# RichardZJM/lammps-mtp-kokkos

Measured on AMD Instinct MI355X. Metric: atom-steps/s (64k-atom W, level-16 MTP), higher is better.
Workload: dtype f64; 1 GPU; 65536-atom BCC W (a=3.165 A, +-0.05 A jitter, seed 777), W_L16.mtp (B=130 T=894 S=116 A=332 R=8 Mu=4 C=149), rc=5 A, full list 7 A, eflag=1 vflag=1; atoms=65536, potential=W_L16.mtp, parallelism=single GPU, atoms_rank0=65536, list_entries_rank0=5802796

## Files before the change

lammps_mtp_kokkos_amd/csrc/mtp_potential.cpp:

```cpp
#include "mtp_potential.hpp"

#include "../../include/mtp_mi355x.h"

#include <algorithm>
#include <cassert>
#include <cerrno>
#include <cmath>
#include <cstdio>
#include <cstdlib>
#include <cstring>
#include <stdexcept>

#include <unistd.h>

namespace {

struct ParseError {
  int code;
  std::string msg;
};

class LineReader {
 public:
  explicit LineReader(FILE *fp) : fp_(fp), buf_(1024) {}
// ... 80 lines not shown
    if (key != kw) throw ParseError{MTP_ERR_PARSE, msg};
  }
};

void parse_text(FILE *fp, bool want_selection, mtp_potential &p)
{
  LineReader rd(fp);
  Cursor c{rd, {}, {}, {}};

  c.advance(kSeps);
  if (c.key != "MTP") throw ParseError{MTP_ERR_FORMAT, "Only MTP potential files are accepted."};
  {
    std::string ver;
    if (!rd.next(ver) || ver != "version = 1.1.0\n")
      throw ParseError{MTP_ERR_FORMAT, "MTP file must have version \"1.1.0\""};
  }
  c.advance(kSeps);
  if (c.key == "potential_name") {
    std::string w;
    p.potential_name = c.tok.next(w) ? w : "";
    c.advance(kSeps);
  }
  p.scaling = 1.0;
  if (c.key == "scaling") {
    p.scaling = c.tok.real();
    c.advance(kSeps);
  }
  c.expect("species_count", "Error reading MTP file. Species count not found.");
  p.species_count = c.tok.integer();
  if (p.species_count < 1) throw ParseError{MTP_ERR_PARSE, "species_count must be positive"};

  c.advance(kSeps);
  if (c.key == "potential_tag") {
    std::string w;
    p.potential_tag = c.tok.next(w) ? w : "";
    c.advance(kSeps);
  }
  c.expect("radial_basis_type", "Error reading MTP file. No radial basis set type is specified.");
  {
    std::string ty = c.tok.word();
    if (ty != "RBChebyshev")
      throw ParseError{MTP_ERR_UNSUPPORTED,
                       "Error reading MTP file. The specified radial basis set type, " + ty + ", was not found.."};
  }
  c.advance(kSeps);
  if (c.key == "scaling") {
    (void) c.tok.real();
    c.advance(kSeps);
  }
  if (c.key != "min_val" && c.key != "min_dist")
    throw ParseError{MTP_ERR_PARSE, "Error in reading MTP file. Cannot read lower cutoff."};
  p.min_cutoff = c.tok.real();
  c.advance(kSeps);
  if (c.key != "max_val" && c.key != "max_dist")
    throw ParseError{MTP_ERR_PARSE, "Error in reading MTP file. Cannot read upper cutoff."};
  p.max_cutoff = c.tok.real();
  c.advance(kSeps);
  c.expect("radial_basis_size", "Error in reading MTP file. Cannot read radial basis set size.");
  p.radial_basis_size = c.tok.integer();

  c.advance(kSeps);
  c.expect("radial_funcs_count", "Error in reading MTP file. Cannot read radial function count.");
  p.radial_func_count = c.tok.integer();
  c.advance(kSeps);
  if (c.key != "radial_coeffs") {
    if (c.key == "magnetic_basis_type")
      throw ParseError{MTP_ERR_UNSUPPORTED, "Magnetic basis is currently not supported."};
    throw ParseError{MTP_ERR_PARSE, "Error in reading MTP file. Cannot read radial coeffs count."};
  }
  const int Sp = p.species_count, R = p.radial_basis_size, Mu = p.radial_func_count;
  if (R < 1 || Mu < 1) throw ParseError{MTP_ERR_PARSE, "radial basis sizes must be positive"};
  p.radial_basis_coeffs.assign((size_t) Sp * Sp * Mu * R, 0.0);
  p.setflag.assign((size_t) (Sp + 1) * (Sp + 1), 0);
  for (int blk = 0; blk < Sp * Sp; blk++) {
    if (!rd.next(c.line)) throw ParseError{MTP_ERR_EOF, "Unexpected end of MTP file."};
    Tokens hdr(c.line, kSepsDash);
    int t1 = hdr.integer(), t2 = hdr.integer();
    if (t1 < 0 || t2 < 0 || t1 >= Sp || t2 >= Sp)
      throw ParseError{MTP_ERR_PARSE, "radial_coeffs block names a species outside species_count"};
    p.setflag[(size_t) (t1 + 1) * (Sp + 1) + t2 + 1] = 1;
    double *dst = &p.radial_basis_coeffs[(size_t) (t1 * Sp + t2) * Mu * R];
    for (int mu = 0; mu < Mu; mu++) {
      if (!rd.next(c.line)) throw ParseError{MTP_ERR_EOF, "Unexpected end of MTP file."};
      Tokens row(c.line, kSepsBrace);
      for (int ri = 0; ri < R; ri++) dst[mu * R + ri] = row.real();
    }
  }
  c.advance(kSeps);
  c.expect("alpha_moments_count", "Error reading MTP file. Alpha moment count not found.");
  p.alpha_moment_count = c.tok.integer();
  c.advance(kSeps);
  c.expect("alpha_index_basic_count", "Error reading MTP file. Alpha moment count not found.");
  p.alpha_index_basic_count = c.tok.integer();
  const int B = p.alpha_index_basic_count;
  if (B < 1) throw ParseError{MTP_ERR_TABLE, "alpha_index_basic_count must be positive"};

  rd.set_bufsize((size_t) B * 20 + 20);
  c.advance(kSepsBrace);
  c.expect("alpha_index_basic", "Error reading MTP file. Alpha index basic not found.");
  p.alpha_index_basic.resize((size_t) B * 4);
  int mu_max = 0, rank_max = 0;
  for (int i = 0; i < B; i++) {
    int32_t *q = &p.alpha_index_basic[4 * (size_t) i];
    for (int j = 0; j < 4; j++) q[j] = c.tok.integer();
    mu_max = std::max(mu_max, (int) q[0]);
    rank_max = std::max(rank_max, (int) (q[1] + q[2] + q[3]));
  }
  if (mu_max != Mu - 1) throw ParseError{MTP_ERR_TABLE, "Wrong number of radial functions specified!"};
  p.max_alpha_index_basic = rank_max + 1;

  c.advance(kSeps);
  c.expect("alpha_index_times_count", "Error reading MTP file. Alpha index times count not found.");
  p.alpha_index_times_count = c.tok.integer();
  const int T = p.alpha_index_times_count;
  rd.set_bufsize((size_t) std::max(T, 0) * 32 + 20);
  c.advance(kSepsBrace);
  c.expect("alpha_index_times", "Error reading MTP file. Alpha index times not found.");
  p.alpha_index_times.resize((size_t) std::max(T, 0) * 4);
  for (size_t i = 0; i < p.alpha_index_times.size(); i++) p.alpha_index_times[i] = c.tok.integer();

  c.advance(kSeps);
  c.expect("alpha_scalar_moments", "Error reading MTP file. Alpha scalar moment count not found.");
  p.alpha_scalar_count = c.tok.integer();
  const int S = p.alpha_scalar_count;
  c.advance(kSepsBrace);
  c.expect("alpha_moment_mapping", "Error reading MTP file. Alpha moment mappings not found.");
  p.alpha_moment_mapping.resize((size_t) S);
  for (int i = 0; i < S; i++) p.alpha_moment_mapping[i] = c.tok.integer();
  c.advance(kSepsBrace);
  c.expect("species_coeffs", "Error reading MTP file. Species coefficients not found.");
  p.species_coeffs.resize((size_t) Sp);
  for (int i = 0; i < Sp; i++) p.species_coeffs[i] = c.tok.real();
  c.advance(kSepsBrace);
  c.expect("moment_coeffs", "Error reading MTP file. Moment coefficients not found.");
  p.linear_coeffs.resize((size_t) S);
  for (int i = 0; i < S; i++) p.linear_coeffs[i] = c.tok.real();

  p.coeff_count = Sp * Sp * Mu * R + Sp + S;

  if (!want_selection) return;
  rd.ignore_comments = false;
  std::string ln;
  if (!rd.next(ln)) {
    p.selection_absent = true;
    throw ParseError{MTP_ERR_SELECTION,
                     "No selection state found! Consider training/retraining or disabling extrapolation!"};
  }
  {
    Tokens t(ln, kSeps);
    std::string w;
    if (!t.next(w) || w != "#MVS_v1.1")
      throw ParseError{MTP_ERR_SELECTION,
                       "Error in reading MTP file selection state. Please verify MVS version is #MVS_v1.1!"};
  }
  rd.ignore_comments = true;
  int energy_weight = 0, site_en_weight = 0;
  static const char *names[5] = {"energy_weight", "force_weight", "stress_weight", "site_en_weight",
                                 "weight_scaling"};
  for (int w = 0; w < 5; w++) {
    c.advance(kSeps);
    if (c.key != names[w])
      throw ParseError{MTP_ERR_SELECTION, std::string("Error in reading MTP file, ") + names[w]};
    if (w == 0) energy_weight = (int) c.tok.real();
    if (w == 3) site_en_weight = (int) c.tok.real();
  }
  if (energy_weight + site_en_weight > 1)
    throw ParseError{MTP_ERR_MODE,
                     "Error, the MTP currently only supports configuration mode (energy_weight=1) or "
                     "neighbourhood mode (site_en_weight=1). Please retrain the MTP with the correct modes!"};
  p.configuration_mode = (energy_weight == 1);
  const size_t n = (size_t) p.coeff_count * p.coeff_count;
  p.active_set.resize(n);
  p.inverse_active_set.resize(n);
  fgetc(fp);
  p.selection_offset = std::ftell(fp);
  if (fread(p.active_set.data(), sizeof(double), n, fp) != n ||
      fread(p.inverse_active_set.data(), sizeof(double), n, fp) != n)
    throw ParseError{MTP_ERR_IO, "Unexpected end of file while reading the active set"};
  p.has_selection = true;
}

}

int mtp_parse_file(const char *path, bool want_selection, mtp_potential &pot, std::string &err)
{
  const int rc = mtp_parse_text_file(path, want_selection, pot, err);
  return rc == MTP_OK ? pot.finalize(err) : rc;
}

int mtp_parse_text_file(const char *path, bool want_selection, mtp_potential &pot, std::string &err)
{
  FILE *fp = std::fopen(path, "rb");
  if (!fp) {
    err = std::string("Cannot open potential file ") + path + ": " + std::strerror(errno);
    return MTP_ERR_IO;
  }
  int rc = MTP_OK;
  try {
    parse_text(fp, want_selection, pot);
  } catch (const ParseError &e) {
    err = e.msg;
    rc = e.code;
  } catch (const std::exception &e) {
    err = e.what();
    rc = MTP_ERR_PARSE;
  }
  std::fclose(fp);
  return rc;
}

void mtp_build_coeff_tables(const mtp_potential &p, const double *radial, const double *species, const double *moments,
                            mtp_coeff_tables &out)
{
  const int A = p.alpha_moment_count, S = p.alpha_scalar_count;
  const std::vector<int32_t> &perm = p.moment_perm;
  const double *lin = moments ? moments : p.linear_coeffs.data();
  const double *ra = radial ? radial : p.radial_basis_coeffs.data();
  const double *sp = species ? species : p.species_coeffs.data();
  out.radial.assign(ra, ra + p.radial_basis_coeffs.size());
  out.species.assign(sp, sp + p.species_coeffs.size());
  auto is_leaf = [&](int m) { return perm[(size_t) m] >= p.stored_moment_count; };
  std::vector<int> last((size_t) A, -1);
  for (int i = 0; i < S; i++) last[(size_t) p.alpha_moment_mapping[(size_t) i]] = i;
  out.seed_val.clear();
  for (int m = 0; m < A; m++)
    if (last[(size_t) m] >= 0 && !is_leaf(m)) out.seed_val.push_back(lin[last[(size_t) m]]);
  std::vector<double> c_energy((size_t) A, 0.0), c_seed((size_t) A, 0.0);
  out.e_lin.clear();
  for (int i = 0; i < S; i++) {
    const int m = p.alpha_moment_mapping[(size_t) i], ml = perm[(size_t) m];
    if (is_leaf(m)) {
      c_energy[(size_t) ml] += lin[i];
      c_seed[(size_t) ml] = lin[i];
    } else {
      out.e_lin.push_back(lin[i]);
    }
  }
  const size_t leaf_row0 = (size_t) p.level_offset[(size_t) p.normal_levels];
  const size_t nleaf_rows = p.rows_by_level.size() - leaf_row0;
  out.leaf_cf.assign(nleaf_rows, 0.0);
  out.leaf_cb.assign(nleaf_rows, 0.0);
  for (size_t r = 0; r < nleaf_rows; r++) {
    const MtpRow &row = p.rows_by_level[leaf_row0 + r];
    if (row.mult == 0) continue;
    out.leaf_cf[r] = c_energy[(size_t) row.a3] * row.mult;
    out.leaf_cb[r] = c_seed[(size_t) row.a3] * row.mult;
  }
}

int mtp_check_compatible(const mtp_potential &a, const mtp_potential &b, bool want_selection, std::string &err)
{
  auto differ = [&](const std::string &name, const std::string &x, const std::string &y) {
    err = "the new file differs in " + name + ": " + y + ", the loaded potential has " + x;
    return (int) MTP_ERR_UNSUPPORTED;
  };
  auto num = [](double v) {
    char t[40];
    std::snprintf(t, sizeof t, "%.17g", v);
    return std::string(t);
  };
#define MTP_SAME_INT(field, name) \
  if (a.field != b.field) return differ(name, std::to_string(a.field), std::to_string(b.field))
#define MTP_SAME_REAL(field, name) \
  if (!(a.field == b.field)) return differ(name, num(a.field), num(b.field))
  MTP_SAME_REAL(scaling, "scaling");
  MTP_SAME_INT(species_count, "species_count");
  MTP_SAME_REAL(min_cutoff, "min_dist");
  MTP_SAME_REAL(max_cutoff, "max_dist");
  MTP_SAME_INT(radial_basis_size, "radial_basis_size");
  MTP_SAME_INT(radial_func_count, "radial_funcs_count");
  MTP_SAME_INT(alpha_moment_count, "alpha_moments_count");
  MTP_SAME_INT(alpha_index_basic_count, "alpha_index_basic_count");
  MTP_SAME_INT(alpha_index_times_count, "alpha_index_times_count");
  MTP_SAME_INT(alpha_scalar_count, "alpha_scalar_moments");
#undef MTP_SAME_INT
#undef MTP_SAME_REAL
  auto table = [&](const char *name, const std::vector<int32_t> &x, const std::vector<int32_t> &y, size_t width) {
    if (x.size() != y.size()) return differ(name, std::to_string(x.size()) + " entries", std::to_string(y.size()) + " entries");
    for (size_t k = 0; k < x.size(); k++)
      if (x[k] != y[k])
        return differ(std::string(name) + "[" + std::to_string(k / width) + (width > 1 ? "][" + std::to_string(k % width) + "]" : "]"),
                      std::to_string(x[k]), std::to_string(y[k]));
    return (int) MTP_OK;
  };
  int rc = table("alpha_index_basic", a.alpha_index_basic, b.alpha_index_basic, 4);
  if (rc == MTP_OK) rc = table("alpha_index_times", a.alpha_index_times, b.alpha_index_times, 4);
  if (rc == MTP_OK) rc = table("alpha_moment_mapping", a.alpha_moment_mapping, b.alpha_moment_mapping, 1);
  if (rc != MTP_OK) return rc;
  if (want_selection) {
    const char *modes[2] = {"neighbourhood (site_en_weight = 1)", "configuration (energy_weight = 1)"};
    if (a.coeff_count != b.coeff_count) return differ("coeff_count", std::to_string(a.coeff_count), std::to_string(b.coeff_count));
    if (a.has_selection != b.has_selection)
      return differ("selection state", a.has_selection ? "present" : "absent", b.has_selection ? "present" : "absent");
    if (a.configuration_mode != b.configuration_mode)
      return differ("selection mode", modes[a.configuration_mode ? 1 : 0], modes[b.configuration_mode ? 1 : 0]);
  }
  return MTP_OK;
}

namespace {

struct ScheduleOptions {
  bool leaves, renumber, debug_banks;
  int bank_rounds = -1, bank_scale = -1, refine_programs = -1;
};

ScheduleOptions read_options()
{
  ScheduleOptions o;
  o.leaves = !std::getenv("MTP_NO_LEAF");
  o.renumber = !std::getenv("MTP_NO_RENUMBER");
  o.debug_banks = std::getenv("MTP_DEBUG_BANKS") != nullptr;
  if (const char *e = std::getenv("MTP_BANK_ROUNDS")) o.bank_rounds = std::max(0, std::atoi(e));
  if (const char *e = std::getenv("MTP_BANK_SCALE")) o.bank_scale = std::max(1, std::atoi(e));
  if (const char *e = std::getenv("MTP_REFINE_PROGRAMS")) o.refine_programs = std::atoi(e) != 0;
  return o;
}

struct Lcg {
  uint64_t state;
  uint32_t operator()() { return (uint32_t) ((state = state * 6364136223846793005ull + 1442695040888963407ull) >> 33); }
};

int refuse(std::string &err, int code, const char *msg)
{
  err = msg;
  return code;
}

int validate(const mtp_potential &p, std::string &err)
{
  const int A = p.alpha_moment_count, B = p.alpha_index_basic_count, T = p.alpha_index_times_count;
  if (A < B) return refuse(err, MTP_ERR_TABLE, "alpha_moments_count is smaller than alpha_index_basic_count");
  for (int i = 0; i < B; i++) {
    const int32_t *q = &p.alpha_index_basic[4 * (size_t) i];
    if (q[0] < 0 || q[1] < 0 || q[2] < 0 || q[3] < 0)
      return refuse(err, MTP_ERR_TABLE, "negative entry in alpha_index_basic");
    if (q[1] > 15 || q[2] > 15 || q[3] > 15)
      return refuse(err, MTP_ERR_LIMIT, "alpha_index_basic exponent above 15 is not supported");
  }
  if (p.max_alpha_index_basic > 12)
    return refuse(err, MTP_ERR_LIMIT, "tensor rank above 11 is not supported by this build");
  for (int k = 0; k < T; k++) {
    const int32_t *q = &p.alpha_index_times[4 * (size_t) k];
    for (int j : {0, 1, 3})
      if (q[j] < 0 || q[j] >= A)
        return refuse(err, MTP_ERR_TABLE, "alpha_index_times refers to a moment outside alpha_moments_count");
  }
  for (int m : p.alpha_moment_mapping)
    if (m < 0 || m >= A)
      return refuse(err, MTP_ERR_TABLE, "alpha_moment_mapping refers to a moment outside alpha_moments_count");
  for (int i = 0; i < B; i++)
    if (p.alpha_index_basic[4 * (size_t) i] > 15)
      return refuse(err, MTP_ERR_LIMIT, "radial function index above 15 is not supported");
  return MTP_OK;
}

int build_slots(mtp_potential &p, std::string &err)
{
  const int B = p.alpha_index_basic_count, P = p.max_alpha_index_basic, Mu = p.radial_func_count;
  p.slot_of.assign((size_t) Mu * P, -1);
  for (int i = 0; i < B; i++) {
    const int32_t *q = &p.alpha_index_basic[4 * (size_t) i];
    p.slot_of[(size_t) q[0] * P + (q[1] + q[2] + q[3])] = -2;
  }
  p.slot_count = 0;
  p.slot_coef_off.clear();
  p.slot_mu.clear();
  p.coef_total = 0;
  for (int nu = 0; nu < 14; nu++) {
    p.deg_first[nu] = p.slot_count;
    p.deg_coef[nu] = p.coef_total;
    if (nu >= P) continue;
    for (int mu = 0; mu < Mu; mu++)
      if (p.slot_of[(size_t) mu * P + nu] == -2) {
        p.slot_of[(size_t) mu * P + nu] = p.slot_count++;
        p.slot_coef_off.push_back(p.coef_total);
        p.slot_mu.push_back(mu);
        p.coef_total += nu == 0 ? 1 : 3 * (nu * (nu + 1) / 2);
      }
  }
  if (p.slot_count > 256) return refuse(err, MTP_ERR_LIMIT, "more than 256 distinct (mu, nu) radial slots");
  p.basic_pack.resize((size_t) B);
  for (int i = 0; i < B; i++) {
    const int32_t *q = &p.alpha_index_basic[4 * (size_t) i];
    const int s = p.slot_of[(size_t) q[0] * P + (q[1] + q[2] + q[3])];
    p.basic_pack[i] = s | (q[1] << 8) | (q[2] << 12) | (q[3] << 16) | (q[0] << 20);
  }
  if (p.coef_total > 65534)
    return refuse(err, MTP_ERR_LIMIT,
                  "derivative-polynomial coefficient blocks above 65534 entries are not supported by this build");
  p.basic_tgt.assign((size_t) 2 * B, 0);
  std::vector<int> hits((size_t) p.coef_total, 0);
  for (int i = 0; i < B; i++) {
    const int32_t *q = &p.alpha_index_basic[4 * (size_t) i];
    const int a = q[1], b = q[2], c = q[3], j = b + c, nu = a + j, C = nu * (nu + 1) / 2;
    const int base = p.slot_coef_off[(size_t) (p.basic_pack[i] & 255)];
    uint32_t tx = 0xffffu, ty = 0xffffu, tz = 0xffffu, fa = (uint32_t) a;
    if (nu == 0) {
      tx = (uint32_t) base;
      fa = 1;
    }
    if (a > 0) tx = (uint32_t) (base + j * (j + 1) / 2 + c);
    if (b > 0) ty = (uint32_t) (base + C + (j - 1) * j / 2 + c);
    if (c > 0) tz = (uint32_t) (base + 2 * C + (j - 1) * j / 2 + c - 1);
    for (uint32_t t : {tx, ty, tz})
      if (t != 0xffffu) hits[t]++;
    p.basic_tgt[2 * (size_t) i] = (int32_t) (tx | (ty << 16));
    p.basic_tgt[2 * (size_t) i + 1] = (int32_t) (tz | (fa << 16) | ((uint32_t) b << 20) | ((uint32_t) c << 24));
  }
  p.coef_dense = 1;
  for (int t = 0; t < p.coef_total; t++) {
    if (hits[t] > 1) return refuse(err, MTP_ERR_TABLE, "alpha_index_basic lists the same (mu, a, b, c) twice");
    if (hits[t] == 0) p.coef_dense = 0;
  }
  return MTP_OK;
}

int build_blocks(mtp_potential &p, std::string &err)
{
  const int B = p.alpha_index_basic_count, P = p.max_alpha_index_basic, slot_count = p.slot_count;
  std::vector<int> basic_of((size_t) slot_count * 16 * 16 * 16, -1);
  for (int i = 0; i < B; i++) {
    const int32_t *q = &p.alpha_index_basic[4 * (size_t) i];
    basic_of[(((size_t) (p.basic_pack[i] & 255) * 16 + q[1]) * 16 + q[2]) * 16 + q[3]] = i;
  }
  p.fwd_blocks.clear();
  p.fwd_block_count = 0;
  std::vector<int> covered((size_t) B, 0);
  for (int j = 0; j < P; j++) {
    std::vector<std::pair<int, int>> heads, tails;
    for (int nu = j; nu < P; nu++)
      for (int sidx = p.deg_first[nu]; sidx < p.deg_first[nu + 1]; sidx++) heads.push_back({sidx, nu - j});
    for (int c = 0; c <= j; c++) tails.push_back({j - c, c});
    for (size_t h0 = 0; h0 < heads.size(); h0 += 3)
      for (size_t t0 = 0; t0 < tails.size(); t0 += 3) {
        int32_t w[8] = {0, 0, 0, 0, 0, 0, 0, 0};
        int16_t kk[10];
        for (int e = 0; e < 10; e++) kk[e] = -1;
        bool any = false;
        for (int h = 0; h < 3 && h0 + h < heads.size(); h++) {
          w[0] |= heads[h0 + h].first << (8 * h);
          w[1] |= heads[h0 + h].second << (4 * h);
        }
        for (int t = 0; t < 3 && t0 + t < tails.size(); t++) {
          w[1] |= tails[t0 + t].first << (12 + 4 * t);
          w[2] |= tails[t0 + t].second << (4 * t);
        }
        for (int h = 0; h < 3 && h0 + h < heads.size(); h++)
          for (int t = 0; t < 3 && t0 + t < tails.size(); t++) {
            const int k = basic_of[(((size_t) heads[h0 + h].first * 16 + heads[h0 + h].second) * 16 +
                                    tails[t0 + t].first) * 16 + tails[t0 + t].second];
            if (k >= 0) {
              kk[3 * h + t] = (int16_t) k;
              covered[k]++;
              any = true;
            }
          }
        if (!any) continue;
        std::memcpy(&w[3], kk, sizeof(int16_t) * 10);
        p.fwd_blocks.insert(p.fwd_blocks.end(), w, w + 8);
        p.fwd_block_count++;
      }
  }
  for (int i = 0; i < B; i++)
    if (covered[i] != 1)
      return refuse(err, MTP_ERR_TABLE, "internal: basic moment not covered exactly once by the head x tail blocks");
  return MTP_OK;
}

int build_blocks5(mtp_potential &p, std::string &err)
{
  const int B = p.alpha_index_basic_count, P = p.max_alpha_index_basic, slot_count = p.slot_count;
  std::vector<int> basic_of((size_t) slot_count * 16 * 16 * 16, -1);
  for (int i = 0; i < B; i++) {
    const int32_t *q = &p.alpha_index_basic[4 * (size_t) i];
    basic_of[(((size_t) (p.basic_pack[i] & 255) * 16 + q[1]) * 16 + q[2]) * 16 + q[3]] = i;
  }
  p.fwd5_blocks.clear();
  p.fwd5_block_count = 0;
  std::vector<int> covered((size_t) B, 0);
  typedef std::pair<int, int> Pair;
  for (int j = 0; j < P; j++) {
    std::vector<Pair> heads, tails;
    auto basic = [&](const Pair &h, const Pair &t) {
      return basic_of[(((size_t) h.first * 16 + h.second) * 16 + t.first) * 16 + t.second];
    };
    {
      std::vector<Pair> all_heads, all_tails;
      for (int nu = j; nu < P; nu++)
        for (int sidx = p.deg_first[nu]; sidx < p.deg_first[nu + 1]; sidx++) all_heads.push_back({sidx, nu - j});
      for (int c = 0; c <= j; c++) all_tails.push_back({j - c, c});
      for (const Pair &h : all_heads)
        if (std::any_of(all_tails.begin(), all_tails.end(), [&](const Pair &t) { return basic(h, t) >= 0; })) heads.push_back(h);
      for (const Pair &t : all_tails)
        if (std::any_of(heads.begin(), heads.end(), [&](const Pair &h) { return basic(h, t) >= 0; })) tails.push_back(t);
    }
    auto cut = [&](int nh, int nt, std::vector<int32_t> *out) {
      int count = 0;
      for (size_t h0 = 0; h0 < heads.size(); h0 += nh)
        for (size_t t0 = 0; t0 < tails.size(); t0 += nt) {
          const int hf[3] = {0, 1, 2}, tf[3] = {3, 4, 2};
          int32_t w[8] = {0, 0, 0, 0, 0, 0, 0, 0};
          int16_t kk[6] = {-1, -1, -1, -1, -1, -1};
          bool any = false;
          for (int h = 0; h < nh && h0 + h < heads.size(); h++) w[hf[h]] |= heads[h0 + h].first | (heads[h0 + h].second << 16);
          for (int t = 0; t < nt && t0 + t < tails.size(); t++) w[tf[t]] |= tails[t0 + t].first | (tails[t0 + t].second << 16);
          if (nh == 3) w[2] |= (int32_t) 0x80000000u;
          for (int h = 0; h < nh && h0 + h < heads.size(); h++)
            for (int t = 0; t < nt && t0 + t < tails.size(); t++) {
              const int k = basic(heads[h0 + h], tails[t0 + t]);
              if (k < 0) continue;
              const int e = h < 2 && t < 2 ? 2 * h + t : nh == 3 ? 4 + t : 4 + h;
              kk[e] = (int16_t) k;
              if (out) covered[k]++;
              any = true;
            }
          if (!any) continue;
          count++;
          if (out) {
            std::memcpy(&w[5], kk, sizeof kk);
            out->insert(out->end(), w, w + 8);
          }
        }
      return count;
    };
    if (heads.empty()) continue;
    const bool wide = cut(3, 2, nullptr) <= cut(2, 3, nullptr);
    p.fwd5_block_count += wide ? cut(3, 2, &p.fwd5_blocks) : cut(2, 3, &p.fwd5_blocks);
  }
  for (int i = 0; i < B; i++)
    if (covered[i] != 1)
      return refuse(err, MTP_ERR_TABLE, "internal: basic moment not covered exactly once by the five-factor blocks");
  return MTP_OK;
}

std::vector<char> find_leaves(const mtp_potential &p, bool enabled)
{
  const int A = p.alpha_moment_count, B = p.alpha_index_basic_count, T = p.alpha_index_times_count;
  std::vector<char> leaf((size_t) A, 0);
  if (!enabled) return leaf;
  std::vector<char> is_factor((size_t) A, 0), is_target((size_t) A, 0);
  std::vector<int> last_write((size_t) A, -1);
  for (int k = 0; k < T; k++) {
    const int32_t *q = &p.alpha_index_times[4 * (size_t) k];
    is_factor[q[0]] = is_factor[q[1]] = 1;
    is_target[q[3]] = 1;
    last_write[q[3]] = k;
  }
  for (int m = B; m < A; m++) leaf[m] = is_target[m] && !is_factor[m];
  for (int k = 0; k < T; k++) {
    const int32_t *q = &p.alpha_index_times[4 * (size_t) k];
    if (leaf[q[3]] && (last_write[q[0]] > k || last_write[q[1]] > k)) leaf[q[3]] = 0;
  }
  return leaf;
}

void build_levels(mtp_potential &p, const std::vector<char> &leaf)
{
  const int A = p.alpha_moment_count, T = p.alpha_index_times_count;
  std::vector<int> wlevel((size_t) A, 0), rlevel((size_t) A, 0);
  std::vector<int> lvl((size_t) T, 0);
  int nlev = 0;
  for (int k = 0; k < T; k++) {
    const int32_t *q = &p.alpha_index_times[4 * (size_t) k];
    if (leaf[q[3]]) continue;
    int l = std::max(wlevel[q[0]], wlevel[q[1]]) + 1;
    l = std::max(l, rlevel[q[3]] + 1);
    lvl[k] = l;
    wlevel[q[3]] = std::max(wlevel[q[3]], l);
    rlevel[q[0]] = std::max(rlevel[q[0]], l);
    rlevel[q[1]] = std::max(rlevel[q[1]], l);
    nlev = std::max(nlev, l);
  }
  p.normal_levels = nlev;
  nlev++;
  for (int k = 0; k < T; k++)
    if (leaf[p.alpha_index_times[4 * (size_t) k + 3]]) lvl[k] = nlev;
  p.level_offset.assign((size_t) nlev + 1, 0);
  for (int k = 0; k < T; k++) p.level_offset[lvl[k]]++;
  for (int l = 1; l <= nlev; l++) p.level_offset[l] += p.level_offset[l - 1];
  std::vector<int32_t> cur((size_t) nlev + 1, 0);
  for (int l = 1; l <= nlev; l++) cur[l] = p.level_offset[l - 1];
  p.rows_by_level.assign((size_t) T, MtpRow{0, 0, 0, 0});
  for (int k = 0; k < T; k++) {
    const int32_t *q = &p.alpha_index_times[4 * (size_t) k];
    p.rows_by_level[cur[lvl[k]]++] = MtpRow{q[0], q[1], q[2], q[3]};
  }
}

void order_rows(mtp_potential &p)
{
  const int nlev = p.normal_levels + 1;
  for (int l = 1; l <= nlev; l++) {
    const int b = p.level_offset[l - 1], e = p.level_offset[l];
    const int n = e - b;
    if (n <= 16) continue;
    std::vector<MtpRow> pool(p.rows_by_level.begin() + b, p.rows_by_level.begin() + e), out;
    std::vector<char> used((size_t) n, 0);
    out.reserve((size_t) n);
    int remaining = n, scan_from = 0;
    while (remaining > 0) {
      int rd0[32], rd1[32], rd3[32];
      for (int h = 0; h < 2 && remaining > 0; h++) {
        if (h == 0)
          for (int q = 0; q < 32; q++) rd0[q] = rd1[q] = rd3[q] = -1;
        int at0[16], at1[16], at3[16];
        for (int q = 0; q < 16; q++) at0[q] = at1[q] = at3[q] = -1;
        for (int slot = 0; slot < 16 && remaining > 0; slot++) {
          int best = -1, best_cost = 1 << 30;
          int seen = 0;
          for (int k = scan_from; k < n && seen < 256; k++) {
            if (used[k]) continue;
            seen++;
            const MtpRow &r = pool[k];
            int cost = 0;
            cost += (rd0[r.a0 & 31] >= 0 && rd0[r.a0 & 31] != r.a0);
            cost += (rd1[r.a1 & 31] >= 0 && rd1[r.a1 & 31] != r.a1);
            if (l < nlev) {
              cost += (rd3[r.a3 & 31] >= 0 && rd3[r.a3 & 31] != r.a3);
              cost += 2 * (at3[r.a3 & 15] >= 0);
            }
            cost += (at0[r.a0 & 15] >= 0) + (at1[r.a1 & 15] >= 0);
            if (cost < best_cost) {
              best_cost = cost;
              best = k;
              if (cost == 0) break;
            }
          }
          assert(best >= 0);
          const MtpRow &r = pool[best];
          used[best] = 1;
          remaining--;
          while (scan_from < n && used[scan_from]) scan_from++;
          rd0[r.a0 & 31] = r.a0;
          rd1[r.a1 & 31] = r.a1;
          rd3[r.a3 & 31] = r.a3;
          at0[r.a0 & 15] = r.a0;
          at1[r.a1 & 15] = r.a1;
          at3[r.a3 & 15] = r.a3;
          out.push_back(r);
        }
      }
    }
    std::copy(out.begin(), out.end(), p.rows_by_level.begin() + b);
  }
}

void pad_levels(mtp_potential &p, const std::vector<char> &leaf)
{
  const int nlev = p.normal_levels + 1;
  std::vector<int> stored;
  for (int m = 0; m < p.alpha_moment_count; m++)
    if (!leaf[m]) stored.push_back(m);
  if (stored.empty()) stored.push_back(0);
  std::vector<MtpRow> padded;
  std::vector<int32_t> off((size_t) nlev + 1, 0);
  for (int l = 1; l <= nlev; l++) {
    const int b = p.level_offset[l - 1], e = p.level_offset[l];
    padded.insert(padded.end(), p.rows_by_level.begin() + b, p.rows_by_level.begin() + e);
    while ((int) padded.size() % 64 != 0) {
      const int t = stored[(size_t) ((int) padded.size() % 64) % stored.size()];
      padded.push_back(MtpRow{t, t, 0, t});
    }
    off[l] = (int32_t) padded.size();
  }
  p.rows_by_level.swap(padded);
  p.level_offset.swap(off);
}

void number_moments(mtp_potential &p, const std::vector<char> &leaf)
{
  const int A = p.alpha_moment_count, B = p.alpha_index_basic_count;
  int nstored = B;
  for (int m = B; m < A; m++) nstored += !leaf[m];
  p.stored_moment_count = nstored;
  p.moment_perm.resize((size_t) A);
  int next_stored = B, next_leaf = nstored;
  for (int m = 0; m < A; m++) p.moment_perm[m] = m < B ? m : (leaf[m] ? next_leaf++ : next_stored++);
}

const int kWRead[3] = {2, 2, 1}, kWAdd[3] = {1, 1, 1};
int pen(int n) { return n > 1 ? n - 1 : 0; }

struct BankModel {
  const mtp_potential &p;
  int leaf_row0;
  int group_cost(int r0, int grp) const
  {
    const int nbk = grp, *w3 = grp == 32 ? kWRead : kWAdd;
    const bool distinct = grp == 32;
    int c = 0;
    for (int st = 0; st < (r0 >= leaf_row0 ? 2 : 3); st++) {
      int seen[32], ns = 0;
      uint8_t h[32] = {0};
      for (int r = r0; r < r0 + grp; r++) {
        const MtpRow &row = p.rows_by_level[(size_t) r];
        const int m = p.moment_perm[st == 0 ? row.a0 : (st == 1 ? row.a1 : row.a3)];
        bool dup = false;
        if (distinct)
          for (int q = 0; q < ns; q++) dup |= seen[q] == m;
        if (!dup) {
          seen[ns++] = m;
          h[m % nbk]++;
        }
      }
      for (int b = 0; b < nbk; b++) c += w3[st] * pen(h[b]);
    }
    return c;
  }
  long long total(int grp) const
  {
    long long c = 0;
    for (size_t r0 = 0; r0 < p.rows_by_level.size(); r0 += grp) c += group_cost((int) r0, grp);
    return c;
  }
};

void renumber_round(mtp_potential &p, const BankModel &model, const std::vector<char> &leaf,
                    const std::vector<int> cls_members[3], Lcg &next, int bank_scale)
{
  const int A = p.alpha_moment_count, B = p.alpha_index_basic_count;
  const std::vector<MtpRow> &rows = p.rows_by_level;
  struct Access {
    int nbk, w;
  };
  std::vector<Access> acc;
  std::vector<std::vector<std::pair<int, int>>> occ((size_t) A);
  std::vector<uint8_t> hist;
  auto add_accesses = [&](int grp) {
    const int nbk = grp, *w3 = grp == 32 ? kWRead : kWAdd;
    const bool distinct = grp == 32;
    const int ngroups = (int) rows.size() / grp;
    for (int g = 0; g < ngroups; g++)
      for (int st = 0; st < (grp * g >= model.leaf_row0 ? 2 : 3); st++) {
        const int id = (int) acc.size();
        acc.push_back({nbk, w3[st]});
        hist.resize(hist.size() + 32, 0);
        for (int r = grp * g; r < grp * g + grp; r++) {
          const MtpRow &row = rows[(size_t) r];
          const int m = st == 0 ? row.a0 : (st == 1 ? row.a1 : row.a3);
          auto &o = occ[(size_t) m];
          if (!o.empty() && o.back().first == id) {
            if (distinct) continue;
            o.back().second++;
          } else {
            o.push_back({id, 1});
          }
          hist[(size_t) id * 32 + (p.moment_perm[m] % nbk)]++;
        }
      }
  };
  add_accesses(32);
  add_accesses(16);
  auto mult_in = [&](int m, int id) {
    const auto &o = occ[(size_t) m];
    auto it = std::lower_bound(o.begin(), o.end(), std::make_pair(id, 0));
    return it != o.end() && it->first == id ? it->second : 0;
  };
  auto move_delta = [&](int m, int from, int to, int other) {
    int d = 0;
    for (const auto &e : occ[(size_t) m]) {
      const int id = e.first, k = e.second, k2 = mult_in(other, id);
      if (k2 > 0 && m > other) continue;
      const int f = from % acc[(size_t) id].nbk, t = to % acc[(size_t) id].nbk;
      if (f == t) continue;
      const uint8_t *h = &hist[(size_t) id * 32];
      d += acc[(size_t) id].w * (pen(h[f] - k + k2) + pen(h[t] + k - k2) - pen(h[f]) - pen(h[t]));
    }
    return d;
  };
  auto apply_move = [&](int m, int from, int to, int other) {
    for (const auto &e : occ[(size_t) m]) {
      const int id = e.first, k = e.second, k2 = mult_in(other, id);
      if (k2 > 0 && m > other) continue;
      const int f = from % acc[(size_t) id].nbk, t = to % acc[(size_t) id].nbk;
      if (f == t) continue;
      hist[(size_t) id * 32 + f] = (uint8_t) (hist[(size_t) id * 32 + f] - k + k2);
      hist[(size_t) id * 32 + t] = (uint8_t) (hist[(size_t) id * 32 + t] + k - k2);
    }
  };
  const long long trials = bank_scale * std::min<long long>(200ll * A, 300000ll);
  for (long long t = 0; t < trials; t++) {
    int m1 = (int) (next() % (uint32_t) A);
    if ((next() & 3) != 0) {
      const MtpRow &pr = rows[next() % (uint32_t) rows.size()];
      const uint32_t st = next() % 3u;
      m1 = st == 0 ? pr.a0 : (st == 1 ? pr.a1 : pr.a3);
    }
    const std::vector<int> &cls = cls_members[m1 < B ? 0 : (leaf[m1] ? 2 : 1)];
    if (cls.size() < 2) continue;
    const int m2 = cls[next() % (uint32_t) cls.size()];
    if (m1 == m2) continue;
    const int p1 = p.moment_perm[m1], p2 = p.moment_perm[m2];
    if (move_delta(m1, p1, p2, m2) + move_delta(m2, p2, p1, m1) >= 0) continue;
    apply_move(m1, p1, p2, m2);
    apply_move(m2, p2, p1, m1);
    std::swap(p.moment_perm[m1], p.moment_perm[m2]);
  }
}

void swap_rows_round(mtp_potential &p, const BankModel &model, Lcg &next, int bank_scale)
{
  std::vector<MtpRow> &rows = p.rows_by_level;
  const int nlev2 = (int) p.level_offset.size() - 1;
  const long long rtrials = bank_scale * std::min<long long>(100ll * (long long) rows.size(), 250000ll);
  for (long long t = 0; t < rtrials; t++) {
    const int l = (int) (next() % (uint32_t) nlev2);
    const int b = p.level_offset[l], n = p.level_offset[l + 1] - b;
    if (n < 2) continue;
    int r1 = b + (int) (next() % (uint32_t) n);
    for (int tries = 0; tries < 4 && model.group_cost(r1 / 16 * 16, 16) == 0; tries++)
      r1 = b + (int) (next() % (uint32_t) n);
    const int r2 = b + (int) (next() % (uint32_t) n);
    if (r1 / 16 == r2 / 16) continue;
    auto local = [&]() {
      int c = model.group_cost(r1 / 16 * 16, 16) + model.group_cost(r2 / 16 * 16, 16);
      c += model.group_cost(r1 / 32 * 32, 32);
      if (r1 / 32 != r2 / 32) c += model.group_cost(r2 / 32 * 32, 32);
      return c;
    };
    const int c0 = local();
    std::swap(rows[(size_t) r1], rows[(size_t) r2]);
    if (local() >= c0) std::swap(rows[(size_t) r1], rows[(size_t) r2]);
  }
}

void report_banks(const mtp_potential &p, const BankModel &model, long long cost_before, int bank_rounds,
                  int bank_scale)
{
  const std::vector<MtpRow> &rows = p.rows_by_level;
  const long long cr = model.total(32), ca = model.total(16);
  long long same_addr[3] = {0, 0, 0}, same_bank[3] = {0, 0, 0};
  for (size_t r0 = 0; r0 < rows.size(); r0 += 16)
    for (int st = 0; st < ((int) r0 >= model.leaf_row0 ? 2 : 3); st++) {
      int ids[16][16], nid[16] = {0}, h[16] = {0};
      for (size_t r = r0; r < r0 + 16; r++) {
        const MtpRow &row = rows[r];
        const int m = p.moment_perm[st == 0 ? row.a0 : (st == 1 ? row.a1 : row.a3)], b = m % 16;
        h[b]++;
        int q = 0;
        while (q < nid[b] && ids[b][q] != m) q++;
        if (q == nid[b]) ids[b][nid[b]++] = m;
      }
      for (int b = 0; b < 16; b++) {
        same_addr[st] += h[b] - nid[b];
        same_bank[st] += pen(h[b]) - (h[b] - nid[b]);
      }
    }
  std::fprintf(stderr, "mtp: LDS bank model of the product passes: %lld -> %lld extra cycles per atom (reads %lld, adds %lld); "
                       "%d head x tail blocks, %d rounds x %d\n", cost_before, cr + ca, cr, ca, p.fwd_block_count, bank_rounds, bank_scale);
  std::fprintf(stderr, "mtp:   adds, same address / other address on the bank: D[a0] %lld / %lld, D[a1] %lld / %lld, M[a3] %lld / %lld\n",
               same_addr[0], same_bank[0], same_addr[1], same_bank[1], same_addr[2], same_bank[2]);
}

void search_banks(mtp_potential &p, const std::vector<char> &leaf, const ScheduleOptions &opt)
{
  std::vector<int> cls_members[3];
  for (int m = 0; m < p.alpha_moment_count; m++)
    cls_members[m < p.alpha_index_basic_count ? 0 : (leaf[m] ? 2 : 1)].push_back(m);
  const BankModel model{p, p.level_offset[(size_t) p.normal_levels]};
  const long long cost_before = model.total(32) + model.total(16);
  const bool row_per_lane = p.fwd_block_count <= 32;
  const int bank_rounds = opt.bank_rounds >= 0 ? opt.bank_rounds : (row_per_lane ? 8 : 2);
  const int bank_scale = opt.bank_scale >= 1 ? opt.bank_scale : (row_per_lane ? 4 : 1);
  Lcg next{0x9E3779B97F4A7C15ull};
  for (int round = 0; round < bank_rounds; round++) {
    renumber_round(p, model, leaf, cls_members, next, bank_scale);
    swap_rows_round(p, model, next, bank_scale);
  }
  if (opt.debug_banks) report_banks(p, model, cost_before, bank_rounds, bank_scale);
}

void relabel(mtp_potential &p, const std::vector<char> &leaf)
{
  const int A = p.alpha_moment_count, B = p.alpha_index_basic_count, S = p.alpha_scalar_count;
  const std::vector<int32_t> &perm = p.moment_perm;
  for (MtpRow &row : p.rows_by_level) {
    row.a0 = perm[row.a0];
    row.a1 = perm[row.a1];
    row.a3 = perm[row.a3];
  }
  std::vector<int> last((size_t) A, -1);
  for (int i = 0; i < S; i++) last[p.alpha_moment_mapping[i]] = i;
  p.seed_idx.clear();
  for (int m = 0; m < A; m++) {
    assert((leaf[m] != 0) == (perm[m] >= p.stored_moment_count));
    if (last[m] >= 0 && !leaf[m]) p.seed_idx.push_back(perm[m]);
  }
  p.e_map.clear();
  for (int i = 0; i < S; i++)
    if (!leaf[p.alpha_moment_mapping[i]]) p.e_map.push_back(perm[p.alpha_moment_mapping[i]]);
  mtp_coeff_tables ct;
  mtp_build_coeff_tables(p, nullptr, nullptr, nullptr, ct);
  p.seed_val.swap(ct.seed_val);
  p.e_lin.swap(ct.e_lin);
  p.leaf_cf.swap(ct.leaf_cf);
  p.leaf_cb.swap(ct.leaf_cb);
  p.mapping_lds.resize((size_t) S);
  for (int i = 0; i < S; i++) p.mapping_lds[i] = perm[p.alpha_moment_mapping[i]];
  p.basic_pack_lds.assign((size_t) B, 0);
  std::vector<int32_t> tgt((size_t) 2 * B, 0);
  for (int i = 0; i < B; i++) {
    p.basic_pack_lds[(size_t) perm[i]] = p.basic_pack[i];
    tgt[2 * (size_t) perm[i]] = p.basic_tgt[2 * (size_t) i];
    tgt[2 * (size_t) perm[i] + 1] = p.basic_tgt[2 * (size_t) i + 1];
  }
  p.basic_tgt.swap(tgt);
  for (int blk = 0; blk < p.fwd_block_count; blk++) {
    int16_t kk[10];
    std::memcpy(kk, &p.fwd_blocks[(size_t) 8 * blk + 3], sizeof kk);
    for (int16_t &k : kk)
      if (k >= 0) k = (int16_t) perm[k];
    std::memcpy(&p.fwd_blocks[(size_t) 8 * blk + 3], kk, sizeof kk);
  }
  for (int blk = 0; blk < p.fwd5_block_count; blk++) {
    int16_t kk[6];
    std::memcpy(kk, &p.fwd5_blocks[(size_t) 8 * blk + 5], sizeof kk);
    for (int16_t &k : kk)
      if (k >= 0) k = (int16_t) perm[k];
    std::memcpy(&p.fwd5_blocks[(size_t) 8 * blk + 5], kk, sizeof kk);
  }
}


struct ProgramLevel {
  std::vector<MtpRow> &prog;
  size_t base;
  int G, cs;
  MtpRow &op(int g, int u, int lane) const { return prog[base + ((size_t) g * cs + u) * 64 + lane]; }
  bool real_chunk(int g, int lane) const
  {
    for (int u = 0; u < cs; u++)
      if (op(g, u, lane).mult != 0) return true;
    return false;
  }
};

void refine_program(const ProgramLevel &lv)
{
  const int G = lv.G, cs = lv.cs;
  int hot = 0;
  auto read_cost = [&](int g, int u, int half, int which) {
    int first[32], extra[32][7], mx = 0;
    uint8_t n[32] = {0};
    for (int lane = 32 * half; lane < 32 * half + 32; lane++) {
      const MtpRow &o = lv.op(g, u, lane);
      if (o.mult == 0) continue;
      const int a = which ? o.a1 : o.a0, b = a & 31;
      bool dup = false;
      if (n[b] > 0) {
        dup = first[b] == a;
        for (int k = 0; k + 1 < n[b] && k < 7 && !dup; k++) dup = extra[b][k] == a;
      }
      if (!dup) {
        if (n[b] == 0) first[b] = a;
        else if (n[b] - 1 < 7) extra[b][n[b] - 1] = a;
        n[b]++;
        if (n[b] > mx) {
          mx = n[b];
          hot = lane;
        }
      }
    }
    return mx > 1 ? mx - 1 : 0;
  };
  auto add_cost = [&](int g, int q) {
    uint8_t h[16] = {0};
    int mx = 0;
    for (int lane = 16 * q; lane < 16 * q + 16; lane++)
      if (lv.real_chunk(g, lane) && ++h[lv.op(g, 0, lane).a3 & 15] > mx) {
        mx = h[lv.op(g, 0, lane).a3 & 15];
        hot = lane;
      }
    return mx > 1 ? 2 * (mx - 1) : 0;
  };
  std::vector<int> rc((size_t) G * cs * 4), ac((size_t) G * 4);
  for (int g = 0; g < G; g++) {
    for (int u = 0; u < cs; u++)
      for (int hw = 0; hw < 4; hw++) rc[((size_t) g * cs + u) * 4 + hw] = read_cost(g, u, hw >> 1, hw & 1);
    for (int q = 0; q < 4; q++) ac[(size_t) g * 4 + q] = add_cost(g, q);
  }
  Lcg next{0xD1B54A32D192ED03ull};
  const long long trials = std::min<long long>(300ll * G * 64, 300000ll);
  for (long long t = 0; t < trials; t++) {
    const int g0 = (int) (next() % (uint32_t) G), u0 = (int) (next() % (uint32_t) cs), hw0 = (int) (next() & 3);
    const bool from_add = (next() & 3) == 0;
    if (from_add) {
      if (ac[(size_t) g0 * 4 + hw0] == 0) continue;
      (void) add_cost(g0, hw0);
    } else {
      if (rc[((size_t) g0 * cs + u0) * 4 + hw0] == 0) continue;
      (void) read_cost(g0, u0, hw0 >> 1, hw0 & 1);
    }
    const int lane0 = hot;
    if (!from_add && cs > 1 && (next() & 1) == 0) {
      const int g = g0, lane = lane0, half = lane >> 5;
      const int u1 = u0, u2 = (int) (next() % (uint32_t) cs);
      if (u1 == u2) continue;
      int before = 0, after = 0;
      for (int w = 0; w < 2; w++) before += rc[((size_t) g * cs + u1) * 4 + 2 * half + w] + rc[((size_t) g * cs + u2) * 4 + 2 * half + w];
      std::swap(lv.op(g, u1, lane), lv.op(g, u2, lane));
      int nc[4];
      for (int w = 0; w < 2; w++) {
        nc[w] = read_cost(g, u1, half, w);
        nc[2 + w] = read_cost(g, u2, half, w);
        after += nc[w] + nc[2 + w];
      }
      if (after > before) {
        std::swap(lv.op(g, u1, lane), lv.op(g, u2, lane));
        continue;
      }
      for (int w = 0; w < 2; w++) {
        rc[((size_t) g * cs + u1) * 4 + 2 * half + w] = nc[w];
        rc[((size_t) g * cs + u2) * 4 + 2 * half + w] = nc[2 + w];
      }
    } else {
      const int g1 = g0, l1 = lane0;
      const int g2 = (int) (next() % (uint32_t) G), l2 = (int) (next() & 63);
      const int h1 = l1 >> 5, h2 = l2 >> 5, q1 = l1 >> 4, q2 = l2 >> 4;
      if (g1 == g2 && q1 == q2) continue;
      const bool same_half = g1 == g2 && h1 == h2;
      int before = ac[(size_t) g1 * 4 + q1] + ac[(size_t) g2 * 4 + q2], after = 0;
      for (int u = 0; u < cs; u++)
        for (int w = 0; w < 2; w++) {
          before += rc[((size_t) g1 * cs + u) * 4 + 2 * h1 + w];
          if (!same_half) before += rc[((size_t) g2 * cs + u) * 4 + 2 * h2 + w];
        }
      for (int u = 0; u < cs; u++) std::swap(lv.op(g1, u, l1), lv.op(g2, u, l2));
      int n1[16], n2[16];
      for (int u = 0; u < cs; u++)
        for (int w = 0; w < 2; w++) {
          n1[2 * u + w] = read_cost(g1, u, h1, w);
          after += n1[2 * u + w];
          if (!same_half) {
            n2[2 * u + w] = read_cost(g2, u, h2, w);
            after += n2[2 * u + w];
          }
        }
      const int a1 = add_cost(g1, q1), a2 = add_cost(g2, q2);
      after += a1 + a2;
      if (after > before) {
        for (int u = 0; u < cs; u++) std::swap(lv.op(g1, u, l1), lv.op(g2, u, l2));
        continue;
      }
      for (int u = 0; u < cs; u++)
        for (int w = 0; w < 2; w++) {
          rc[((size_t) g1 * cs + u) * 4 + 2 * h1 + w] = n1[2 * u + w];
          if (!same_half) rc[((size_t) g2 * cs + u) * 4 + 2 * h2 + w] = n2[2 * u + w];
        }
      ac[(size_t) g1 * 4 + q1] = a1;
      ac[(size_t) g2 * 4 + q2] = a2;
    }
  }
}

void fill_wildcards(const ProgramLevel &lv, int A_st)
{
  for (int g = 0; g < lv.G; g++) {
    for (int u = 0; u < lv.cs; u++)
      for (int half = 0; half < 2; half++) {
        int a0 = 0, a1 = 0;
        for (int lane = 32 * half; lane < 32 * half + 32; lane++)
          if (lv.op(g, u, lane).mult != 0) {
            a0 = lv.op(g, u, lane).a0;
            a1 = lv.op(g, u, lane).a1;
            break;
          }
        for (int lane = 32 * half; lane < 32 * half + 32; lane++)
          if (lv.op(g, u, lane).mult == 0) {
            lv.op(g, u, lane).a0 = a0;
            lv.op(g, u, lane).a1 = a1;
          }
      }
    for (int q = 0; q < 4; q++) {
      bool busy[16] = {false};
      for (int lane = 16 * q; lane < 16 * q + 16; lane++)
        if (lv.real_chunk(g, lane)) busy[lv.op(g, 0, lane).a3 & 15] = true;
      for (int lane = 16 * q; lane < 16 * q + 16; lane++) {
        if (lv.real_chunk(g, lane)) continue;
        int t = lv.op(g, 0, lane).a3;
        for (int m = 0; m < A_st; m++)
          if (!busy[m & 15]) {
            t = m;
            break;
          }
        busy[t & 15] = true;
        for (int u = 0; u < lv.cs; u++) lv.op(g, u, lane).a3 = t;
      }
    }
  }
}

void build_program(const mtp_potential &p, bool reverse, bool refine, std::vector<MtpRow> &prog,
                   std::vector<int32_t> &seg)
{
  const int A = p.alpha_moment_count;
  const int nlev2 = p.normal_levels;
  const int A_st = p.stored_moment_count;
  prog.clear();
  seg.clear();
  for (int li = 0; li < nlev2; li++) {
    const int l = reverse ? nlev2 - 1 - li : li;
    std::vector<std::vector<MtpRow>> by_tgt((size_t) A);
    for (int r = p.level_offset[l]; r < p.level_offset[l + 1]; r++) {
      const MtpRow &row = p.rows_by_level[(size_t) r];
      if (row.mult == 0) continue;
      if (!reverse) {
        by_tgt[(size_t) row.a3].push_back(row);
      } else if (row.a0 == row.a1 && 2 * row.mult <= 32767 && 2 * row.mult >= -32768) {
        by_tgt[(size_t) row.a0].push_back(MtpRow{row.a3, row.a0, 2 * row.mult, row.a0});
      } else {
        by_tgt[(size_t) row.a1].push_back(MtpRow{row.a3, row.a0, row.mult, row.a1});
        by_tgt[(size_t) row.a0].push_back(MtpRow{row.a3, row.a1, row.mult, row.a0});
      }
    }
    int best_cs = 1;
    long long best_cost = -1;
    for (int cs : {1, 2, 4, 8}) {
      long long chunks = 0;
      for (const auto &v : by_tgt) chunks += ((long long) v.size() + cs - 1) / cs;
      const long long groups = (chunks + 63) / 64, cost = groups * cs * 6 + groups * 15;
      if (best_cost < 0 || cost < best_cost) {
        best_cost = cost;
        best_cs = cs;
      }
    }
    const int cs = best_cs;
    struct Chunk {
      int tgt;
      MtpRow op[8];
    };
    std::vector<Chunk> chunks;
    for (int t = 0; t < A; t++) {
      const auto &v = by_tgt[(size_t) t];
      for (size_t b = 0; b < v.size(); b += (size_t) cs) {
        Chunk c;
        c.tgt = t;
        for (int u = 0; u < cs; u++) c.op[u] = b + u < v.size() ? v[b + u] : MtpRow{t, t, 0, t};
        chunks.push_back(c);
      }
    }
    const int ngroups = (int) ((chunks.size() + 63) / 64);
    const int first_block = (int) (prog.size() / 64);
    std::vector<char> used(chunks.size(), 0);
    size_t scan_from = 0;
    for (int g = 0; g < ngroups; g++) {
      int occx[8][2][32], occy[8][2][32], occt[4][16];
      std::fill_n(&occx[0][0][0], 8 * 2 * 32, -1);
      std::fill_n(&occy[0][0][0], 8 * 2 * 32, -1);
      std::fill_n(&occt[0][0], 4 * 16, -1);
      std::vector<MtpRow> blk((size_t) 64 * cs);
      for (int lane = 0; lane < 64; lane++) {
        const int half = lane >> 5, q16 = lane >> 4;
        int best = -1, best_rot = 0, bcost = 1 << 30, seen = 0;
        for (size_t k = scan_from; k < chunks.size() && seen < 128; k++) {
          if (used[k]) continue;
          seen++;
          const Chunk &c = chunks[k];
          const int tcost = 3 * (occt[q16][c.tgt & 15] >= 0);
          for (int rot = 0; rot < cs; rot++) {
            int cost = tcost;
            for (int u = 0; u < cs; u++) {
              const MtpRow &o = c.op[(u + rot) % cs];
              const int bx = occx[u][half][o.a0 & 31], by = occy[u][half][o.a1 & 31];
              cost += (bx >= 0 && bx != o.a0) + (by >= 0 && by != o.a1);
            }
            if (cost < bcost) {
              bcost = cost;
              best = (int) k;
              best_rot = rot;
            }
            if (cost == 0) break;
          }
// ... 435 lines not shown
```

Baseline: 235.5 million atom-steps/s.

## Replace greedy LDS bank-conflict search with simulated annealing over moments and rows

Adds a v2 bank-assignment search that uses simulated annealing, with a cooling schedule of acceptance thresholds, for both the moment renumbering and the row reordering. Row moves now include a0/a1 operand exchange, pair swaps with optional exchange, and 3-cycles, and the best state seen is kept. The goal is fewer LDS bank conflicts in the product passes of the kernel. The cost is a longer one-time setup search. The old greedy search stays available via MTP_BANK_SEARCH=v1 and is still used when there are more than 32 forward blocks.

```diff
diff --git a/lammps_mtp_kokkos_amd/csrc/mtp_potential.cpp b/lammps_mtp_kokkos_amd/csrc/mtp_potential.cpp
--- a/lammps_mtp_kokkos_amd/csrc/mtp_potential.cpp
+++ b/lammps_mtp_kokkos_amd/csrc/mtp_potential.cpp
@@ -406,6 +406,7 @@
 
 struct ScheduleOptions {
   bool leaves, renumber, debug_banks;
+  bool search_v1;
   int bank_rounds = -1, bank_scale = -1, refine_programs = -1;
 };
 
@@ -415,6 +416,8 @@
   o.leaves = !std::getenv("MTP_NO_LEAF");
   o.renumber = !std::getenv("MTP_NO_RENUMBER");
   o.debug_banks = std::getenv("MTP_DEBUG_BANKS") != nullptr;
+  const char *search = std::getenv("MTP_BANK_SEARCH");
+  o.search_v1 = search && std::strcmp(search, "v1") == 0;
   if (const char *e = std::getenv("MTP_BANK_ROUNDS")) o.bank_rounds = std::max(0, std::atoi(e));
   if (const char *e = std::getenv("MTP_BANK_SCALE")) o.bank_scale = std::max(1, std::atoi(e));
   if (const char *e = std::getenv("MTP_REFINE_PROGRAMS")) o.refine_programs = std::atoi(e) != 0;
@@ -821,8 +824,29 @@
   }
 };
 
+constexpr int BANK_ROUNDS_V2 = 4, BANK_SCALE_V2 = 16;
+constexpr int ANNEAL_K0 = 24, ANNEAL_K_STEP = 8, ANNEAL_K1 = 60;
+constexpr int ROW_TRIALS_V2 = 200;
+constexpr long long ROW_TRIALS_MIN = 200000;
+constexpr long long RENUMBER_TRIALS_MIN = 50000;
+
+struct Anneal {
+  int k0, k1, k = -1;
+  uint32_t thr[8] = {0};
+  void at(long long t, long long trials)
+  {
+    const int kk = k0 + (int) ((long long) (k1 - k0) * t / std::max(trials, 1ll));
+    if (kk == k) return;
+    k = kk;
+    uint64_t qk = 1ull << 32, f = 1ull << 31;
+    for (int i = 0; i < k; i++) qk = (qk * 3611622603ull) >> 32;
+    for (int d = 1; d < 8; d++) thr[d] = (uint32_t) (f = (f * qk) >> 32);
+  }
+  bool pass(int d, Lcg &next) const { return d <= 0 || (d < 8 && next() < thr[d]); }
+};
+
 void renumber_round(mtp_potential &p, const BankModel &model, const std::vector<char> &leaf,
-                    const std::vector<int> cls_members[3], Lcg &next, int bank_scale)
+                    const std::vector<int> cls_members[3], Lcg &next, int bank_scale, Anneal *an = nullptr)
 {
   const int A = p.alpha_moment_count, B = p.alpha_index_basic_count;
   const std::vector<MtpRow> &rows = p.rows_by_level;
@@ -884,8 +908,12 @@
       hist[(size_t) id * 32 + t] = (uint8_t) (hist[(size_t) id * 32 + t] + k - k2);
     }
   };
-  const long long trials = bank_scale * std::min<long long>(200ll * A, 300000ll);
+  long long trials = bank_scale * std::min<long long>(200ll * A, 300000ll);
+  if (an) trials = std::max(trials, RENUMBER_TRIALS_MIN);
+  long long cur = 0, best = 0;
+  std::vector<int32_t> best_perm;
   for (long long t = 0; t < trials; t++) {
+    if (an) an->at(t, trials);
     int m1 = (int) (next() % (uint32_t) A);
     if ((next() & 3) != 0) {
       const MtpRow &pr = rows[next() % (uint32_t) rows.size()];
@@ -897,11 +925,19 @@
     const int m2 = cls[next() % (uint32_t) cls.size()];
     if (m1 == m2) continue;
     const int p1 = p.moment_perm[m1], p2 = p.moment_perm[m2];
-    if (move_delta(m1, p1, p2, m2) + move_delta(m2, p2, p1, m1) >= 0) continue;
+    const int delta = move_delta(m1, p1, p2, m2) + move_delta(m2, p2, p1, m1);
+    if (an ? !an->pass(delta, next) : delta >= 0) continue;
+    if (an && delta > 0 && cur == best && best_perm.empty()) best_perm = p.moment_perm;
     apply_move(m1, p1, p2, m2);
     apply_move(m2, p2, p1, m1);
     std::swap(p.moment_perm[m1], p.moment_perm[m2]);
-  }
+    cur += delta;
+    if (cur <= best) {
+      best = cur;
+      best_perm.clear();
+    }
+  }
+  if (!best_perm.empty()) p.moment_perm.swap(best_perm);
 }
 
 void swap_rows_round(mtp_potential &p, const BankModel &model, Lcg &next, int bank_scale)
@@ -930,11 +966,118 @@
   }
 }
 
-void report_banks(const mtp_potential &p, const BankModel &model, long long cost_before, int bank_rounds,
-                  int bank_scale)
+struct RowAnnealer {
+  std::vector<MtpRow> &rows;
+  const std::vector<int32_t> &perm;
+  const int leaf_row0, A;
+  std::vector<uint8_t> hadd, hread, rcnt;
+  std::vector<int> gcost;
+  RowAnnealer(mtp_potential &p, int leaf_row0_)
+      : rows(p.rows_by_level), perm(p.moment_perm), leaf_row0(leaf_row0_), A(p.alpha_moment_count)
+  {
+    hadd.assign(rows.size() / 16 * 3 * 16, 0);
+    hread.assign(rows.size() / 32 * 3 * 32, 0);
+    rcnt.assign(rows.size() / 32 * 3 * (size_t) A, 0);
+    gcost.assign(rows.size() / 16, 0);
+    for (int r = 0; r < (int) rows.size(); r++) (void) put(r, +1);
+  }
+  int put(int r, int s)
+  {
+    const MtpRow &row = rows[(size_t) r];
+    const int m3[3] = {row.a0, row.a1, row.a3};
+    int d = 0;
+    for (int st = 0; st < (r >= leaf_row0 ? 2 : 3); st++) {
+      const int m = m3[st], num = perm[(size_t) m];
+      uint8_t &h = hadd[((size_t) (r / 16) * 3 + st) * 16 + num % 16];
+      const int da = kWAdd[st] * (pen(h + s) - pen(h));
+      h = (uint8_t) (h + s);
+      gcost[(size_t) (r / 16)] += da;
+      d += da;
+      uint8_t &c = rcnt[((size_t) (r / 32) * 3 + st) * A + m];
+      if ((s > 0 ? c : c - 1) == 0) {
+        uint8_t &hr = hread[((size_t) (r / 32) * 3 + st) * 32 + num % 32];
+        d += kWRead[st] * (pen(hr + s) - pen(hr));
+        hr = (uint8_t) (hr + s);
+      }
+      c = (uint8_t) (c + s);
+    }
+    return d;
+  }
+  int place(const int *pos, const MtpRow *now, int n)
+  {
+    int d = 0;
+    for (int i = 0; i < n; i++) d += put(pos[i], -1);
+    for (int i = 0; i < n; i++) rows[(size_t) pos[i]] = now[i];
+    for (int i = 0; i < n; i++) d += put(pos[i], +1);
+    return d;
+  }
+};
+
+void anneal_rows_round(mtp_potential &p, const BankModel &model, Lcg &next, long long trials, Anneal &an)
+{
+  RowAnnealer ra(p, model.leaf_row0);
+  std::vector<MtpRow> &rows = p.rows_by_level;
+  const int nlev2 = (int) p.level_offset.size() - 1;
+  auto exchanged = [](MtpRow r) {
+    std::swap(r.a0, r.a1);
+    return r;
+  };
+  long long cur = 0, best = 0;
+  std::vector<MtpRow> best_rows;
+  for (long long t = 0; t < trials; t++) {
+    an.at(t, trials);
+    const int l = (int) (next() % (uint32_t) nlev2);
+    const int b = p.level_offset[l], n = p.level_offset[l + 1] - b;
+    if (n < 1) continue;
+    int pos[3] = {b + (int) (next() % (uint32_t) n), 0, 0};
+    for (int tries = 0; tries < 4 && ra.gcost[(size_t) (pos[0] / 16)] == 0; tries++) pos[0] = b + (int) (next() % (uint32_t) n);
+    const uint32_t kind = next() % 8u;
+    MtpRow was[3], now[3];
+    int np = 1;
+    if (kind < 2) {
+      if (rows[(size_t) pos[0]].a0 == rows[(size_t) pos[0]].a1) continue;
+    } else {
+      np = kind < 6 ? 2 : 3;
+      for (int i = 1; i < np; i++) pos[i] = b + (int) (next() % (uint32_t) n);
+      if (pos[0] / 16 == pos[1] / 16 || (np == 3 && (pos[2] / 16 == pos[0] / 16 || pos[2] / 16 == pos[1] / 16))) continue;
+    }
+    for (int i = 0; i < np; i++) was[i] = rows[(size_t) pos[i]];
+    if (kind < 2) {
+      now[0] = exchanged(was[0]);
+    } else if (kind < 6) {
+      now[0] = was[1];
+      now[1] = was[0];
+      if (kind >= 4) {
+        const uint32_t which = 1u + next() % 3u;
+        if (which & 1u) now[0] = exchanged(now[0]);
+        if (which & 2u) now[1] = exchanged(now[1]);
+      }
+    } else {
+      now[0] = was[2];
+      now[1] = was[0];
+      now[2] = was[1];
+    }
+    const int delta = ra.place(pos, now, np);
+    if (!an.pass(delta, next)) {
+      (void) ra.place(pos, was, np);
+      continue;
+    }
+    if (delta > 0 && cur == best && best_rows.empty()) {
+      best_rows = rows;
+      for (int i = 0; i < np; i++) best_rows[(size_t) pos[i]] = was[i];
+    }
+    cur += delta;
+    if (cur <= best) {
+      best = cur;
+      best_rows.clear();
+    }
+  }
+  if (!best_rows.empty()) rows.swap(best_rows);
+}
+
+void report_split(const mtp_potential &p, const BankModel &model, const char *when)
 {
   const std::vector<MtpRow> &rows = p.rows_by_level;
-  const long long cr = model.total(32), ca = model.total(16);
   long long same_addr[3] = {0, 0, 0}, same_bank[3] = {0, 0, 0};
   for (size_t r0 = 0; r0 < rows.size(); r0 += 16)
     for (int st = 0; st < ((int) r0 >= model.leaf_row0 ? 2 : 3); st++) {
@@ -952,10 +1095,42 @@
         same_bank[st] += pen(h[b]) - (h[b] - nid[b]);
       }
     }
+  std::fprintf(stderr, "mtp:   %s: reads %lld, adds %lld; adds, same address / other address on the bank: D[a0] %lld / %lld, D[a1] %lld / %lld, M[a3] %lld / %lld\n",
+               when, model.total(32), model.total(16), same_addr[0], same_bank[0], same_addr[1], same_bank[1], same_addr[2],
+               same_bank[2]);
+}
+
+void report_banks(const mtp_potential &p, const BankModel &model, long long cost_before, int bank_rounds,
+                  int bank_scale, bool v1)
+{
+  const std::vector<MtpRow> &rows = p.rows_by_level;
+  const long long cr = model.total(32), ca = model.total(16);
   std::fprintf(stderr, "mtp: LDS bank model of the product passes: %lld -> %lld extra cycles per atom (reads %lld, adds %lld); "
-                       "%d head x tail blocks, %d rounds x %d\n", cost_before, cr + ca, cr, ca, p.fwd_block_count, bank_rounds, bank_scale);
-  std::fprintf(stderr, "mtp:   adds, same address / other address on the bank: D[a0] %lld / %lld, D[a1] %lld / %lld, M[a3] %lld / %lld\n",
-               same_addr[0], same_bank[0], same_addr[1], same_bank[1], same_addr[2], same_bank[2]);
+                       "%d head x tail blocks, %d rounds x %d, search %s\n", cost_before, cr + ca, cr, ca, p.fwd_block_count,
+               bank_rounds, bank_scale, v1 ? "v1" : "v2");
+  report_split(p, model, "after");
+  long long forced_d = 0, forced_m = 0;
+  std::vector<int> uf((size_t) p.alpha_moment_count), ut((size_t) p.alpha_moment_count);
+  for (size_t l = 0; l + 1 < p.level_offset.size(); l++) {
+    const int b = p.level_offset[l], e = p.level_offset[l + 1], groups = (e - b) / 16;
+    std::fill(uf.begin(), uf.end(), 0);
+    std::fill(ut.begin(), ut.end(), 0);
+    for (int r = b; r < e; r++) {
+      uf[(size_t) rows[(size_t) r].a0]++;
+      uf[(size_t) rows[(size_t) r].a1]++;
+      if (r < model.leaf_row0) ut[(size_t) rows[(size_t) r].a3]++;
+    }
+    long long fd = 0, fm = 0;
+    for (int m = 0; m < p.alpha_moment_count; m++) {
+      fd += std::max(0, uf[(size_t) m] - 2 * groups);
+      fm += std::max(0, ut[(size_t) m] - groups);
+    }
+    std::fprintf(stderr, "mtp:   forced same-address adds, %s %d (%d add groups): D[a0] + D[a1] %lld, M[a3] %lld\n",
+                 b >= model.leaf_row0 ? "leaf block" : "level", (int) l + 1, groups, fd, fm);
+    forced_d += fd;
+    forced_m += fm;
+  }
+  std::fprintf(stderr, "mtp:   forced same-address adds in all: D[a0] + D[a1] %lld, M[a3] %lld\n", forced_d, forced_m);
 }
 
 void search_banks(mtp_potential &p, const std::vector<char> &leaf, const ScheduleOptions &opt)
@@ -965,15 +1140,25 @@
     cls_members[m < p.alpha_index_basic_count ? 0 : (leaf[m] ? 2 : 1)].push_back(m);
   const BankModel model{p, p.level_offset[(size_t) p.normal_levels]};
   const long long cost_before = model.total(32) + model.total(16);
+  if (opt.debug_banks) report_split(p, model, "before");
   const bool row_per_lane = p.fwd_block_count <= 32;
-  const int bank_rounds = opt.bank_rounds >= 0 ? opt.bank_rounds : (row_per_lane ? 8 : 2);
-  const int bank_scale = opt.bank_scale >= 1 ? opt.bank_scale : (row_per_lane ? 4 : 1);
+  const bool v1 = opt.search_v1 || !row_per_lane;
+  const int bank_rounds = opt.bank_rounds >= 0 ? opt.bank_rounds : (!row_per_lane ? 2 : (v1 ? 8 : BANK_ROUNDS_V2));
+  const int bank_scale = opt.bank_scale >= 1 ? opt.bank_scale : (!row_per_lane ? 1 : (v1 ? 4 : BANK_SCALE_V2));
   Lcg next{0x9E3779B97F4A7C15ull};
   for (int round = 0; round < bank_rounds; round++) {
-    renumber_round(p, model, leaf, cls_members, next, bank_scale);
-    swap_rows_round(p, model, next, bank_scale);
-  }
-  if (opt.debug_banks) report_banks(p, model, cost_before, bank_rounds, bank_scale);
+    if (v1) {
+      renumber_round(p, model, leaf, cls_members, next, bank_scale);
+      swap_rows_round(p, model, next, bank_scale);
+    } else {
+      Anneal an{ANNEAL_K0 + ANNEAL_K_STEP * round / std::max(bank_rounds - 1, 1), ANNEAL_K1};
+      renumber_round(p, model, leaf, cls_members, next, bank_scale, &an);
+      an.k = -1;
+      const long long row_trials = bank_scale * ROW_TRIALS_V2 * (long long) p.rows_by_level.size();
+      anneal_rows_round(p, model, next, std::max(row_trials, ROW_TRIALS_MIN), an);
+    }
+  }
+  if (opt.debug_banks) report_banks(p, model, cost_before, bank_rounds, bank_scale, v1);
 }
 
 void relabel(mtp_potential &p, const std::vector<char> &leaf)
```

Result: faster. 242.3 million atom-steps/s, median of 6 (+2.9%).
